# niqbal996/triton_client

Hardware: AMD Instinct MI355X
Metric: end-to-end FPS (sensor->detection) YOLOv5n-640 + PointPillars at 1/2/4/8 GPU (higher is better)
Workload: dtype fp32

## Files before the change

### csrc/kernels/conv_hx3.hip

```cpp
#include "tca_mfma.h"

#include <cstdlib>

using namespace tca;

namespace {

struct Hx3Args {
  const float* in_f;
  const float* res_f;
  float* out_f;
  const void* w;
  const float* bias;
  int B, H, W, Cin, ldi, ci_off, Ho, Wo;
  int N, ldo, co_off, ldr, r_off;
  int act;
  const unsigned char* occ;
  const unsigned char* uni;
  const float* uni_val;
  int uni_min;
};

template <int TH, int BN, int WM, int WN, bool CM>
__device__ __forceinline__ void hx3_epilogue(const Hx3Args& a, unsigned char* smem,
                                             const f32x4 (&acc)[TH / WM][BN / WN / 16], int b, int oy0, int ox0,
                                             int n0) {
  constexpr int BM = TH * 16, NT = WM * WN * 64, FM = TH / WM, FN = BN / WN / 16, LD = BN;
  static_assert(BN % 64 == 0, "the quad swizzle needs >= 16 quads per row");
  const int tid = threadIdx.x, lane = tid & 63, wid = tid >> 6;
  const int wm = wid / WN, wn = wid % WN, fr = lane & 15, fq = lane >> 4;
  float* st = reinterpret_cast<float*>(smem);
  auto quad = [](int ml, int q) { return ml * LD + ((q ^ (ml & 15)) << 2); };
  const int act = a.act & 15;
  const bool post_res = (a.act & 16) != 0 && a.res_f != nullptr;
  const int eact = post_res ? 0 : act;
#pragma unroll
  for (int j = 0; j < FN; ++j) {
    const int nl = (wn * FN + j) * 16 + fq * 4;
    const float4 bv = a.bias ? *reinterpret_cast<const float4*>(a.bias + n0 + nl) : make_float4(0.f, 0.f, 0.f, 0.f);
#pragma unroll
    for (int i = 0; i < FM; ++i) {
      const int ml = (wm * FM + i) * 16 + fr;
      float4 q = make_float4(acc[i][j][0] + bv.x, acc[i][j][1] + bv.y, acc[i][j][2] + bv.z, acc[i][j][3] + bv.w);
      if (eact == 1) {
        q.x = fmaxf(q.x, 0.f); q.y = fmaxf(q.y, 0.f); q.z = fmaxf(q.z, 0.f); q.w = fmaxf(q.w, 0.f);
      } else if (eact != 0) {
        q.x = act_fn(q.x, eact); q.y = act_fn(q.y, eact); q.z = act_fn(q.z, eact); q.w = act_fn(q.w, eact);
      }
      *reinterpret_cast<float4*>(st + quad(ml, nl >> 2)) = q;
    }
  }
  __syncthreads();
  constexpr int V8 = BN / 8;
  for (int id = tid; id < BM * V8; id += NT) {
    const int ml = id / V8, c8 = (id - (id / V8) * V8) * 8;
    const int oy = oy0 + (CM ? (ml & 15) : ml / 16), ox = ox0 + (CM ? ml / 16 : (ml & 15)), n = n0 + c8;
    if (oy >= a.Ho || ox >= a.Wo) continue;
    float v[8];
    const float4 v0 = *reinterpret_cast<const float4*>(st + quad(ml, c8 >> 2));
    const float4 v1 = *reinterpret_cast<const float4*>(st + quad(ml, (c8 >> 2) + 1));
    v[0] = v0.x; v[1] = v0.y; v[2] = v0.z; v[3] = v0.w; v[4] = v1.x; v[5] = v1.y; v[6] = v1.z; v[7] = v1.w;
    const long pix = ((long)b * a.Ho + oy) * a.Wo + ox;
    if (a.res_f) {
      float r[8];
      pair_join8(a.res_f + pix * a.ldr + a.r_off + n, r);
#pragma unroll
      for (int e = 0; e < 8; ++e) v[e] = post_res ? act_fn(v[e] + r[e], act) : v[e] + r[e];
    }
    const long o = pix * a.ldo + a.co_off + n;
    if (a.act & 32) {
      *reinterpret_cast<float4*>(a.out_f + o) = make_float4(v[0], v[1], v[2], v[3]);
      *reinterpret_cast<float4*>(a.out_f + o + 4) = make_float4(v[4], v[5], v[6], v[7]);
      continue;
    }
    uint4 hi, lo;
    pair_split8(v, hi, lo);
    *reinterpret_cast<uint4*>(a.out_f + o) = hi;
    *reinterpret_cast<uint4*>(a.out_f + o + 4) = lo;
  }
}

template <int BM, int BN, bool CM, int NT>
__device__ __forceinline__ bool uni_tile_store(const Hx3Args& a, int b, int oy0, int ox0, int n0) {
  const int tid = threadIdx.x;
  bool bad = false;
  for (int ml = tid; ml < BM; ml += NT) {
    const int oy = oy0 + (CM ? (ml & 15) : ml / 16), ox = ox0 + (CM ? ml / 16 : (ml & 15));
    if (oy < a.Ho && ox < a.Wo) bad |= a.uni[((long)b * a.Ho + oy) * a.Wo + ox] < a.uni_min;
  }
  if (__syncthreads_or(bad)) return false;
  constexpr int Q = BN / 4;
  for (int id = tid; id < BM * Q; id += NT) {
    const int ml = id / Q, q = id - (id / Q) * Q;
    const int oy = oy0 + (CM ? (ml & 15) : ml / 16), ox = ox0 + (CM ? ml / 16 : (ml & 15));
    if (oy >= a.Ho || ox >= a.Wo) continue;
    const long o = (((long)b * a.Ho + oy) * a.Wo + ox) * a.ldo + a.co_off + n0 + q * 4;
    *reinterpret_cast<uint4*>(a.out_f + o) = *reinterpret_cast<const uint4*>(a.uni_val + n0 + q * 4);
  }
  return true;
}

template <int V> struct IC { static constexpr int value = V; };

template <int TH, int BN, int WM, int WN, bool CM, int HB, int MINW = 2, bool PAIRS = false>
__global__ void __launch_bounds__(WM * WN * 64, MINW) conv_hx3_kernel(Hx3Args a) {
  constexpr int TW = 16, BM = TH * TW, NW = WM * WN, NT = NW * 64;
  constexpr int FM = TH / WM, FN = BN / WN / 16;
  static_assert(TH % WM == 0 && BN % (WN * 16) == 0 && FN >= 1, "tiles");
  static_assert(HB == 1 || HB == 2, "halo buffers");
  constexpr int HWD = TW + 2, HP = (TH + 2) * HWD;
  constexpr int HPIECES = HP * 8;
  constexpr int HPL = (HPIECES + NT - 1) / NT;
  constexpr int HBYTES = HP * 128;
  constexpr int EPI = BM * (BN + 4) * 4;
  constexpr int LDS = (HB * HBYTES > EPI) ? HB * HBYTES : EPI;
  __shared__ __attribute__((aligned(1024))) unsigned char smem[LDS];

  const int tid = threadIdx.x, lane = tid & 63, wid = tid >> 6;
  const int wm = wid / WN, wn = wid % WN;
  constexpr int EX = CM ? TH : TW, EY = CM ? TW : TH;
  const int tx_n = (a.Wo + EX - 1) / EX, ty_n = (a.Ho + EY - 1) / EY;
  const int nmt = a.B * ty_n * tx_n, nnt = a.N / BN, nwg = nmt * nnt;
  int bid = blockIdx.x;
  {
    const int xcd = bid & 7, q = nwg >> 3, r = nwg & 7;
    if (nwg >= 8) bid = (xcd < r ? xcd * (q + 1) : r * (q + 1) + (xcd - r) * q) + (bid >> 3);
  }
  const int mt = bid / nnt, nt = bid - mt * nnt;
  const int b = mt / (ty_n * tx_n), rem = mt - b * (ty_n * tx_n);
  const int oy0 = (rem / tx_n) * EY, ox0 = (rem - (rem / tx_n) * tx_n) * EX;
  const int n0 = nt * BN;

  if (a.uni && uni_tile_store<TH * TW, BN, CM, NT>(a, b, oy0, ox0, n0)) return;

  const __amdgpu_buffer_rsrc_t rin = __builtin_amdgcn_make_buffer_rsrc(
      (void*)a.in_f, (short)0, a.B * a.H * a.W * a.ldi * 4, 0x00020000);
  unsigned h_off[HPL];
  int h_lds[HPL];
#pragma unroll
  for (int k = 0; k < HPL; ++k) {
    const int q = tid + k * NT, p = q >> 3, piece = q & 7;
    h_off[k] = kOutOfRange;
    h_lds[k] = -1;
    if (q < HPIECES) {
      const int u = p / HWD, v = p - (p / HWD) * HWD;
      const int hy = CM ? v : u, hx = CM ? u : v;
      const int iy = oy0 - 1 + hy, ix = ox0 - 1 + hx;
      if ((unsigned)iy < (unsigned)a.H && (unsigned)ix < (unsigned)a.W)
        h_off[k] = (unsigned)((((b * a.H + iy) * a.W + ix) * a.ldi + a.ci_off) * 4 + piece * 16);
      h_lds[k] = p * 128 + ((piece ^ hswz(v)) << 4);
    }
  }
  typedef unsigned int u32x4 __attribute__((ext_vector_type(4)));
  u32x4 hreg[HPL];
  auto halo_load = [&](int c) {
#pragma unroll
    for (int k = 0; k < HPL; ++k) hreg[k] = __builtin_amdgcn_raw_buffer_load_b128(rin, h_off[k], c * 128, 0);
  };
  auto halo_write = [&](int buf) {
    unsigned char* dst = smem + buf * HBYTES;
#pragma unroll
    for (int k = 0; k < HPL; ++k)
      if (k + 1 < HPL || h_lds[k] >= 0) *reinterpret_cast<u32x4*>(dst + h_lds[k]) = hreg[k];
  };

  const int NG = a.N / 16, g0 = (n0 + wn * FN * 16) / 16;
  const __bf16* wf = reinterpret_cast<const __bf16*>(a.w) + (long)g0 * 1024 + lane * 8;
  const int nc = a.Cin / 32;
  auto wload = [&](int ks, bf16x8 (&dst)[FN][2]) {
    const __bf16* p = wf + (long)ks * NG * 1024;
#pragma unroll
    for (int j = 0; j < FN; ++j) {
      dst[j][0] = *reinterpret_cast<const bf16x8*>(p + j * 1024);
      dst[j][1] = *reinterpret_cast<const bf16x8*>(p + j * 1024 + 512);
    }
  };

  f32x4 acc[FM][FN];
#pragma unroll
  for (int i = 0; i < FM; ++i)
#pragma unroll
    for (int j = 0; j < FN; ++j) acc[i][j] = f32x4{0.f, 0.f, 0.f, 0.f};

  const int G = 3 * nc;
  auto gload = [&](int gs, bf16x8 (&dst)[3][FN][2]) {
    const int c = gs / 3, kf = gs - (gs / 3) * 3;
#pragma unroll
    for (int kl = 0; kl < 3; ++kl) {
      const int t = CM ? 3 * kf + kl : 3 * kl + kf;
      wload(t * nc + c, dst[kl]);
    }
  };
  bf16x8 wc[3][FN][2], wx[3][FN][2];
  halo_load(0);
  gload(0, wc);
  halo_write(0);
  halo_load(nc > 1 ? 1 : 0);
  asm volatile("s_waitcnt lgkmcnt(0)" ::: "memory");
  __builtin_amdgcn_s_barrier();
  asm volatile("" ::: "memory");

  const int fr = lane & 15, fq = lane >> 4;
  auto group = [&](auto KF, const unsigned char* hb, bf16x8 (&wu)[3][FN][2], bf16x8 (&wl)[3][FN][2], int gs_next) {
    constexpr int kf = decltype(KF)::value;
    gload(gs_next < G ? gs_next : G - 1, wl);
    __builtin_amdgcn_sched_barrier(0);
    const int sw = hswz(kf + fr);
    const unsigned char* colp = hb + (wm * FM) * HWD * 128 + (kf + fr) * 128;
    const int o_hi = ((2 * fq) ^ sw) << 4, o_lo = ((2 * fq + 1) ^ sw) << 4;
#pragma unroll
    for (int L = 0; L < FM + 2; ++L) {
      const bf16x8 ah = *reinterpret_cast<const bf16x8*>(colp + L * HWD * 128 + o_hi);
      const bf16x8 al = *reinterpret_cast<const bf16x8*>(colp + L * HWD * 128 + o_lo);
#pragma unroll
      for (int pr = 0; pr < 3; ++pr) {
#pragma unroll
        for (int kl = 0; kl < 3; ++kl) {
          const int i = L - kl;
          if (i < 0 || i >= FM) continue;
#pragma unroll
          for (int j = 0; j < FN; ++j) {
            const bf16x8& b = pr == 0 ? wu[kl][j][1] : wu[kl][j][0];
            const bf16x8& x = pr == 1 ? al : ah;
            acc[i][j] = __builtin_amdgcn_mfma_f32_16x16x32_bf16(b, x, acc[i][j], 0, 0, 0);
          }
        }
      }
    }
  };
  auto chunk_end = [&](int c) {
    if (c + 1 < nc) {
      if constexpr (HB == 1) {
        asm volatile("s_waitcnt lgkmcnt(0)" ::: "memory");
        __builtin_amdgcn_s_barrier();
        asm volatile("" ::: "memory");
      }
      halo_write(HB == 2 ? (c + 1) & 1 : 0);
      halo_load(c + 2 < nc ? c + 2 : nc - 1);
      asm volatile("s_waitcnt lgkmcnt(0)" ::: "memory");
      __builtin_amdgcn_s_barrier();
      asm volatile("" ::: "memory");
    }
  };
  if constexpr (PAIRS) {
    const unsigned char* hb1 = smem + (HB == 2 ? HBYTES : 0);
    for (int c = 0; c < nc; c += 2) {
      group(IC<0>{}, smem, wc, wx, 3 * c + 1);
      group(IC<1>{}, smem, wx, wc, 3 * c + 2);
      group(IC<2>{}, smem, wc, wx, 3 * c + 3);
      chunk_end(c);
      group(IC<0>{}, hb1, wx, wc, 3 * c + 4);
      group(IC<1>{}, hb1, wc, wx, 3 * c + 5);
      group(IC<2>{}, hb1, wx, wc, 3 * c + 6);
      chunk_end(c + 1);
    }
  } else {
    for (int c = 0; c < nc; ++c) {
      const unsigned char* hb = smem + (HB == 2 ? (c & 1) * HBYTES : 0);
      auto copyw = [&]() {
#pragma unroll
        for (int kl = 0; kl < 3; ++kl)
#pragma unroll
          for (int j = 0; j < FN; ++j) {
            wc[kl][j][0] = wx[kl][j][0];
            wc[kl][j][1] = wx[kl][j][1];
          }
      };
      group(IC<0>{}, hb, wc, wx, 3 * c + 1);
      copyw();
      group(IC<1>{}, hb, wc, wx, 3 * c + 2);
      copyw();
      group(IC<2>{}, hb, wc, wx, 3 * c + 3);
      copyw();
      chunk_end(c);
    }
  }
  asm volatile("s_waitcnt lgkmcnt(0)" ::: "memory");
  __builtin_amdgcn_s_barrier();
  asm volatile("" ::: "memory");

  hx3_epilogue<TH, BN, WM, WN, CM>(a, smem, acc, b, oy0, ox0, n0);
}

template <int G> struct S2Group {
  static constexpr int PL = G >= 3 ? 1 : 0;
  static constexpr int PF = (G == 0 || G == 3) ? 0 : 1;
  static constexpr int FI = (G == 2 || G == 5) ? 1 : 0;
  static constexpr int KF = PF == 0 ? 1 : 2 * FI;
  static constexpr int FOFF = PF == 0 ? 1 : FI;
  static constexpr int NL = PL == 0 ? 1 : 2;
  static constexpr int PH = PL * 2 + PF;
  static constexpr bool LAST_OF_PHASE = G == 0 || G == 2 || G == 3 || G == 5;
  __device__ static constexpr int kl(int li) { return PL == 0 ? 1 : 2 * li; }
  __device__ static constexpr int loff(int li) { return PL == 0 ? 1 : li; }
};

template <int TH, int BN, int WN, bool CM, int MINW, bool OCC>
__global__ void __launch_bounds__(WN * 64, MINW) conv_hx3s2_kernel(Hx3Args a) {
  constexpr int TW = 16, NT = WN * 64;
  constexpr int FM = TH, FN = BN / WN / 16;
  static_assert(BN % (WN * 16) == 0 && FN >= 1, "tiles");
  constexpr int HWD = TW + 1, HP = (TH + 1) * HWD;
  constexpr int HPIECES = HP * 8;
  constexpr int HPL = (HPIECES + NT - 1) / NT;
  constexpr int HBYTES = HP * 128;
  constexpr int EPI = TH * TW * (BN + 4) * 4;
  constexpr int LDS = (2 * HBYTES > EPI) ? 2 * HBYTES : EPI;
  __shared__ __attribute__((aligned(1024))) unsigned char smem[LDS];

  const int tid = threadIdx.x, lane = tid & 63, wn = tid >> 6;
  constexpr int EX = CM ? TH : TW, EY = CM ? TW : TH;
  const int tx_n = (a.Wo + EX - 1) / EX, ty_n = (a.Ho + EY - 1) / EY;
  const int nmt = a.B * ty_n * tx_n, nnt = a.N / BN, nwg = nmt * nnt;
  int bid = blockIdx.x;
  {
    const int xcd = bid & 7, q = nwg >> 3, r = nwg & 7;
    if (nwg >= 8) bid = (xcd < r ? xcd * (q + 1) : r * (q + 1) + (xcd - r) * q) + (bid >> 3);
  }
  const int mt = bid / nnt, nt = bid - mt * nnt;
  const int b = mt / (ty_n * tx_n), rem = mt - b * (ty_n * tx_n);
  const int oy0 = (rem / tx_n) * EY, ox0 = (rem - (rem / tx_n) * tx_n) * EX;
  const int n0 = nt * BN;
  if (a.uni && uni_tile_store<TH * TW, BN, CM, NT>(a, b, oy0, ox0, n0)) return;

  const __amdgpu_buffer_rsrc_t rin = __builtin_amdgcn_make_buffer_rsrc(
      (void*)a.in_f, (short)0, a.B * a.H * a.W * a.ldi * 4, 0x00020000);
  const int pix_b = a.ldi * 4, row_b = a.W * a.ldi * 4;
  const int dl = CM ? pix_b : row_b, df = CM ? row_b : pix_b;
  unsigned h_off[HPL];
  int h_lds[HPL];
  unsigned h_ph[HPL];
#pragma unroll
  for (int k = 0; k < HPL; ++k) {
    const int q = tid + k * NT, p = q >> 3, piece = q & 7;
    h_off[k] = kOutOfRange;
    h_lds[k] = -1;
    h_ph[k] = 0;
    if (q < HPIECES) {
      const int u = p / HWD, v = p - (p / HWD) * HWD;
      const int hy = CM ? v : u, hx = CM ? u : v;
      const int Y = oy0 - 1 + hy, X = ox0 - 1 + hx;
      if (Y >= 0 && X >= 0 && 2 * Y < a.H && 2 * X < a.W) {
        h_off[k] = (unsigned)((((b * a.H + 2 * Y) * a.W + 2 * X) * a.ldi + a.ci_off) * 4 + piece * 16);
#pragma unroll
        for (int ph = 0; ph < 4; ++ph) {
          const int pl = ph >> 1, pf = ph & 1;
          const int iy = 2 * Y + (CM ? pf : pl), ix = 2 * X + (CM ? pl : pf);
          bool ok = iy < a.H && ix < a.W;
          if constexpr (OCC) ok = ok && a.occ[((long)b * a.H + iy) * a.W + ix] != 0;
          h_ph[k] |= ok ? (1u << ph) : 0u;
        }
      }
      h_lds[k] = p * 128 + ((piece ^ hswz(v)) << 4);
    }
  }
  typedef unsigned int u32x4 __attribute__((ext_vector_type(4)));
  u32x4 hreg[2][HPL];
  auto halo_load = [&](int ph, int c, auto SL) {
    constexpr int sl = decltype(SL)::value;
    const int so = c * 128 + (ph >> 1) * dl + (ph & 1) * df;
#pragma unroll
    for (int k = 0; k < HPL; ++k)
      hreg[sl][k] = __builtin_amdgcn_raw_buffer_load_b128(rin, ((h_ph[k] >> ph) & 1u) ? h_off[k] : kOutOfRange, so, 0);
  };
  auto halo_write = [&](int buf, auto SL) {
    constexpr int sl = decltype(SL)::value;
    unsigned char* dst = smem + buf * HBYTES;
#pragma unroll
    for (int k = 0; k < HPL; ++k)
      if (k + 1 < HPL || h_lds[k] >= 0) *reinterpret_cast<u32x4*>(dst + h_lds[k]) = hreg[sl][k];
  };

  const int NG = a.N / 16, g0 = (n0 + wn * FN * 16) / 16;
  const __bf16* wf = reinterpret_cast<const __bf16*>(a.w) + (long)g0 * 1024 + lane * 8;
  const int nc = a.Cin / 32;
  auto wload = [&](int ks, bf16x8 (&dst)[FN][2]) {
    const __bf16* p = wf + (long)ks * NG * 1024;
#pragma unroll
    for (int j = 0; j < FN; ++j) {
      dst[j][0] = *reinterpret_cast<const bf16x8*>(p + j * 1024);
      dst[j][1] = *reinterpret_cast<const bf16x8*>(p + j * 1024 + 512);
    }
  };
  auto gload = [&](auto GC, int c, bf16x8 (&dst)[2][FN][2]) {
    using S = S2Group<decltype(GC)::value>;
#pragma unroll
    for (int li = 0; li < S::NL; ++li) {
      const int t = CM ? 3 * S::KF + S::kl(li) : 3 * S::kl(li) + S::KF;
      wload(t * nc + c, dst[li]);
    }
  };

  f32x4 acc[FM][FN];
#pragma unroll
  for (int i = 0; i < FM; ++i)
#pragma unroll
    for (int j = 0; j < FN; ++j) acc[i][j] = f32x4{0.f, 0.f, 0.f, 0.f};

  if constexpr (OCC) {
    unsigned mine = 0;
#pragma unroll
    for (int k = 0; k < HPL; ++k) mine |= h_ph[k];
    if (!__syncthreads_or(mine != 0u)) {
      hx3_epilogue<TH, BN, 1, WN, CM>(a, smem, acc, b, oy0, ox0, n0);
      return;
    }
  }
  bf16x8 w0[2][FN][2], w1[2][FN][2];
  halo_load(0, 0, IC<0>{});
  gload(IC<0>{}, 0, w0);
  halo_write(0, IC<0>{});
  halo_load(1, 0, IC<1>{});
  halo_load(4 * nc > 2 ? 2 : 4 * nc - 1, 0, IC<0>{});
  asm volatile("s_waitcnt lgkmcnt(0)" ::: "memory");
  __builtin_amdgcn_s_barrier();
  asm volatile("" ::: "memory");

  const int fr = lane & 15, fq = lane >> 4;
  auto phase_end = [&](auto PH, int c) {
    constexpr int ph = decltype(PH)::value;
    const int q = 4 * c + ph;
    if (q + 1 < 4 * nc) {
      halo_write((ph + 1) & 1, IC<(ph + 1) & 1>{});
      const int q3 = q + 3 < 4 * nc ? q + 3 : 4 * nc - 1;
      halo_load(q3 & 3, q3 >> 2, IC<(ph + 1) & 1>{});
      asm volatile("s_waitcnt lgkmcnt(0)" ::: "memory");
      __builtin_amdgcn_s_barrier();
      asm volatile("" ::: "memory");
    }
  };
  auto group = [&](auto GC, int c, bf16x8 (&wu)[2][FN][2], bf16x8 (&wl)[2][FN][2]) {
    constexpr int G = decltype(GC)::value;
    using S = S2Group<G>;
    if constexpr (G < 5) gload(IC<G + 1>{}, c, wl);
    else gload(IC<0>{}, c + 1 < nc ? c + 1 : nc - 1, wl);
    __builtin_amdgcn_sched_barrier(0);
    const unsigned char* hb = smem + (S::PH & 1) * HBYTES;
    const int sw = hswz(S::FOFF + fr);
    const unsigned char* colp = hb + (S::FOFF + fr) * 128;
    const int o_hi = ((2 * fq) ^ sw) << 4, o_lo = ((2 * fq + 1) ^ sw) << 4;
#pragma unroll
    for (int L = (S::NL == 1 ? 1 : 0); L < FM + 1; ++L) {
      const bf16x8 ah = *reinterpret_cast<const bf16x8*>(colp + L * HWD * 128 + o_hi);
      const bf16x8 al = *reinterpret_cast<const bf16x8*>(colp + L * HWD * 128 + o_lo);
#pragma unroll
      for (int pr = 0; pr < 3; ++pr) {
#pragma unroll
        for (int li = 0; li < S::NL; ++li) {
          const int i = L - S::loff(li);
          if (i < 0 || i >= FM) continue;
#pragma unroll
          for (int j = 0; j < FN; ++j) {
            const bf16x8& b = pr == 0 ? wu[li][j][1] : wu[li][j][0];
            const bf16x8& x = pr == 1 ? al : ah;
            acc[i][j] = __builtin_amdgcn_mfma_f32_16x16x32_bf16(b, x, acc[i][j], 0, 0, 0);
          }
        }
      }
    }
    if constexpr (S::LAST_OF_PHASE) phase_end(IC<S::PH>{}, c);
  };
  for (int c = 0; c < nc; ++c) {
    group(IC<0>{}, c, w0, w1);
    group(IC<1>{}, c, w1, w0);
    group(IC<2>{}, c, w0, w1);
    group(IC<3>{}, c, w1, w0);
    group(IC<4>{}, c, w0, w1);
    group(IC<5>{}, c, w1, w0);
  }
  asm volatile("s_waitcnt lgkmcnt(0)" ::: "memory");
  __builtin_amdgcn_s_barrier();
  asm volatile("" ::: "memory");
  hx3_epilogue<TH, BN, 1, WN, CM>(a, smem, acc, b, oy0, ox0, n0);
}


template <int TH, int BN, int WM, int WN, bool CM, int HB, int MINW = 2>
int launch_hx3(const Hx3Args& a, hipStream_t stream) {
  if (a.N % BN) return (int)hipErrorInvalidValue;
  const int ex = CM ? TH : 16, ey = CM ? 16 : TH;
  const int nwg = a.B * ((a.Ho + ey - 1) / ey) * ((a.Wo + ex - 1) / ex) * (a.N / BN);
  if ((a.Cin / 32) % 2 == 0)
    conv_hx3_kernel<TH, BN, WM, WN, CM, HB, MINW, true><<<nwg, WM * WN * 64, 0, stream>>>(a);
  else
    conv_hx3_kernel<TH, BN, WM, WN, CM, HB, MINW, false><<<nwg, WM * WN * 64, 0, stream>>>(a);
  return (int)hipGetLastError();
}

int hx3_launch(const Hx3Args& a, int tile, hipStream_t stream) {
  if (tile == 0) {
    const long rm8 = (long)((a.Wo + 15) / 16 * 16) * ((a.Ho + 7) / 8 * 8);
    const long cm8 = (long)((a.Ho + 15) / 16 * 16) * ((a.Wo + 7) / 8 * 8);
    if (a.N % 128 == 0) tile = cm8 < rm8 ? 2 : 1;
    else if (a.N % 64 == 0) tile = cm8 < rm8 ? 6 : 5;
    else return (int)hipErrorInvalidValue;
  }
  switch (tile) {
    case 1: return launch_hx3<8, 128, 1, 4, false, 2>(a, stream);
    case 2: return launch_hx3<8, 128, 1, 4, true, 2>(a, stream);
    case 3: return launch_hx3<8, 64, 2, 2, false, 2>(a, stream);
    case 4: return launch_hx3<8, 64, 2, 2, true, 2>(a, stream);
    case 5: return launch_hx3<8, 64, 1, 4, false, 2, 3>(a, stream);
    case 6: return launch_hx3<8, 64, 1, 4, true, 2, 3>(a, stream);
    default: return (int)hipErrorInvalidValue;
  }
}


template <int TH, int BN, int WN, bool CM, int MINW>
int launch_hx3s2(const Hx3Args& a, hipStream_t stream) {
  if (a.N % BN) return (int)hipErrorInvalidValue;
  const int ex = CM ? TH : 16, ey = CM ? 16 : TH;
  const int nwg = a.B * ((a.Ho + ey - 1) / ey) * ((a.Wo + ex - 1) / ex) * (a.N / BN);
  if (a.occ) conv_hx3s2_kernel<TH, BN, WN, CM, MINW, true><<<nwg, WN * 64, 0, stream>>>(a);
  else conv_hx3s2_kernel<TH, BN, WN, CM, MINW, false><<<nwg, WN * 64, 0, stream>>>(a);
  return (int)hipGetLastError();
}

int hx3s2_launch(const Hx3Args& a, int tile, hipStream_t stream) {
  if (tile == 0) {
    const long rm8 = (long)((a.Wo + 15) / 16 * 16) * ((a.Ho + 7) / 8 * 8);
    const long cm8 = (long)((a.Ho + 15) / 16 * 16) * ((a.Wo + 7) / 8 * 8);
    if (a.N % 128 == 0) tile = cm8 < rm8 ? 2 : 1;
    else if (a.N % 64 == 0) tile = cm8 < rm8 ? 4 : 3;
    else return (int)hipErrorInvalidValue;
  }
  switch (tile) {
    case 1: return launch_hx3s2<8, 128, 4, false, 2>(a, stream);
    case 2: return launch_hx3s2<8, 128, 4, true, 2>(a, stream);
    case 3: return launch_hx3s2<8, 64, 4, false, 3>(a, stream);
    case 4: return launch_hx3s2<8, 64, 4, true, 3>(a, stream);
    default: return (int)hipErrorInvalidValue;
  }
}

}

TCA_API int tca_conv_hx3p(const float* in, int B, int H, int W, int Cin, int ldi, int ci_off, const void* wfrag,
                          const float* bias, int N, float* out, int ldo, int co_off, int act, const float* res,
                          int ldr, int r_off, int tile, hipStream_t stream) {
  if (B <= 0) return 0;
  if ((Cin & 31) || (ldi & 7) || (ci_off & 7) || (N & 63) || (ldo & 7) || (co_off & 7)) return (int)hipErrorInvalidValue;
  if (res && ((ldr & 7) || (r_off & 7))) return (int)hipErrorInvalidValue;
  Hx3Args a;
  a.in_f = in; a.res_f = res; a.out_f = out; a.w = wfrag; a.bias = bias; a.occ = nullptr;
  a.uni = nullptr; a.uni_val = nullptr; a.uni_min = 0;
  a.B = B; a.H = H; a.W = W; a.Cin = Cin; a.ldi = ldi; a.ci_off = ci_off; a.Ho = H; a.Wo = W;
  a.N = N; a.ldo = ldo; a.co_off = co_off; a.ldr = ldr; a.r_off = r_off; a.act = act;
  if ((long)B * H * W * ldi * 4 >= (1L << 31)) return (int)hipErrorInvalidValue;
  return hx3_launch(a, tile, stream);
}

TCA_API int tca_conv_hx3s2p(const float* in, int B, int H, int W, int Cin, int ldi, int ci_off, const void* wfrag,
                            const float* bias, int N, float* out, int ldo, int co_off, int act, const float* res,
                            int ldr, int r_off, const unsigned char* occ, const unsigned char* uni, int uni_min,
                            const float* uni_val, int tile, hipStream_t stream) {
  if (B <= 0) return 0;
  if ((act & 32) && res) return (int)hipErrorInvalidValue;
  if ((Cin & 31) || (ldi & 7) || (ci_off & 7) || (N & 63) || (ldo & 7) || (co_off & 7)) return (int)hipErrorInvalidValue;
  if (res && ((ldr & 7) || (r_off & 7))) return (int)hipErrorInvalidValue;
  Hx3Args a;
  if (uni && (!uni_val || uni_min < 1 || res)) return (int)hipErrorInvalidValue;
  a.in_f = in; a.res_f = res; a.out_f = out; a.w = wfrag; a.bias = bias; a.occ = occ;
  a.uni = uni; a.uni_val = uni_val; a.uni_min = uni ? uni_min : 0;
  a.B = B; a.H = H; a.W = W; a.Cin = Cin; a.ldi = ldi; a.ci_off = ci_off; a.Ho = (H + 1) / 2; a.Wo = (W + 1) / 2;
  a.N = N; a.ldo = ldo; a.co_off = co_off; a.ldr = ldr; a.r_off = r_off; a.act = act;
  if ((long)B * H * W * ldi * 4 >= (1L << 31)) return (int)hipErrorInvalidValue;
  return hx3s2_launch(a, tile, stream);
}

TCA_API int tca_conv_hx3p_uni(const float* in, int B, int H, int W, int Cin, int ldi, int ci_off, const void* wfrag,
                              const float* bias, int N, float* out, int ldo, int co_off, int act,
                              const unsigned char* uni, int uni_min, const float* uni_val, int tile,
                              hipStream_t stream) {
  if (B <= 0) return 0;
  if ((Cin & 31) || (ldi & 7) || (ci_off & 7) || (N & 63) || (ldo & 7) || (co_off & 7)) return (int)hipErrorInvalidValue;
  if (!uni || !uni_val || uni_min < 1) return (int)hipErrorInvalidValue;
  Hx3Args a;
  a.in_f = in; a.res_f = nullptr; a.out_f = out; a.w = wfrag; a.bias = bias; a.occ = nullptr;
  a.uni = uni; a.uni_val = uni_val; a.uni_min = uni_min;
  a.B = B; a.H = H; a.W = W; a.Cin = Cin; a.ldi = ldi; a.ci_off = ci_off; a.Ho = H; a.Wo = W;
  a.N = N; a.ldo = ldo; a.co_off = co_off; a.ldr = 0; a.r_off = 0; a.act = act;
  if ((long)B * H * W * ldi * 4 >= (1L << 31)) return (int)hipErrorInvalidValue;
  return hx3_launch(a, tile, stream);
}

namespace {

constexpr int UD_TY = 16, UD_TX = 64, UD_MAXR = 7;
static_assert(UD_TX + 2 * UD_MAXR < 128, "u rows are walked 128 columns at a time");

__global__ void __launch_bounds__(256) bev_uniform_depth_kernel(const unsigned char* __restrict__ occ, int H, int W,
                                                                 int Ho, int Wo, int maxd,
                                                                 unsigned char* __restrict__ depth) {
  constexpr int LY = UD_TY + 2 * UD_MAXR, LX = UD_TX + 2 * UD_MAXR;
  constexpr int OY = 2 * LY + 1, OX = 2 * LX + 1;
  __shared__ unsigned char u[LY * LX];
  __shared__ unsigned char os[OY * OX];
  const int b = blockIdx.z, ty0 = blockIdx.y * UD_TY, tx0 = blockIdx.x * UD_TX;
  const int R = maxd - 1;
  const int ry = UD_TY + 2 * R, rx = UD_TX + 2 * R;
  const unsigned char* oc = occ + (long)b * H * W;
  const int iy0 = 2 * (ty0 - R) - 1, ix0 = 2 * (tx0 - R) - 1, oy = 2 * ry + 1, ox = 2 * rx + 1;
  const int lane = threadIdx.x & 63, wv = threadIdx.x >> 6, nw = blockDim.x >> 6;
  for (int r = wv; r < oy; r += nw) {
    const int iy = iy0 + r;
    const bool row_in = (unsigned)iy < (unsigned)H;
    for (int c = lane; c < ox; c += 64) {
      const int ix = ix0 + c;
      os[r * OX + c] = (row_in && (unsigned)ix < (unsigned)W) ? oc[(long)iy * W + ix] : 0;
    }
  }
  __syncthreads();
  for (int id = threadIdx.x; id < ry * 128; id += blockDim.x) {
    const int ly = id >> 7, lx = id & 127;
    if (lx >= rx) continue;
    const int Y = ty0 - R + ly, X = tx0 - R + lx;
    unsigned char good = 0;
    if (Y >= 0 && X >= 0 && Y < Ho && X < Wo) {
      const unsigned char* w = os + (2 * ly) * OX + 2 * lx;
      const unsigned any = w[0] | w[1] | w[2] | w[OX] | w[OX + 1] | w[OX + 2] | w[2 * OX] | w[2 * OX + 1] |
                           w[2 * OX + 2];
      good = any ? 0 : 1;
    }
    u[ly * LX + lx] = good;
  }
  __syncthreads();
  for (int id = threadIdx.x; id < UD_TY * UD_TX; id += blockDim.x) {
    const int py = id / UD_TX, px = id - (id / UD_TX) * UD_TX;
    const int Y = ty0 + py, X = tx0 + px;
    if (Y >= Ho || X >= Wo) continue;
    const int cy = py + R, cx = px + R;
    int d = 0;
    if (u[cy * LX + cx]) {
      d = 1;
      for (int k = 1; k <= R; ++k) {
        bool ok = true;
        for (int t = -k; t <= k && ok; ++t)
          ok = u[(cy - k) * LX + cx + t] && u[(cy + k) * LX + cx + t] && u[(cy + t) * LX + cx - k] &&
               u[(cy + t) * LX + cx + k];
        if (!ok) break;
        d = k + 1;
      }
    }
    depth[((long)b * Ho + Y) * Wo + X] = (unsigned char)d;
  }
}

}

TCA_API int tca_bev_uniform_depth(const unsigned char* occ, int B, int H, int W, int maxd, unsigned char* depth,
                                  hipStream_t stream) {
  if (B <= 0) return 0;
  if (maxd < 1 || maxd > UD_MAXR + 1) return (int)hipErrorInvalidValue;
  const int Ho = (H + 1) / 2, Wo = (W + 1) / 2;
  dim3 grid((unsigned)((Wo + UD_TX - 1) / UD_TX), (unsigned)((Ho + UD_TY - 1) / UD_TY), (unsigned)B);
  bev_uniform_depth_kernel<<<grid, 256, 0, stream>>>(occ, H, W, Ho, Wo, maxd, depth);
  TCA_LAUNCH_CHECK();
}
```

### triton_client_amd/ops/conv.py

```python
from __future__ import annotations

import os

from dataclasses import dataclass
from typing import Optional

import torch
import torch.nn as nn
import torch.nn.functional as F

from .. import _native
from ..models.common import ACT_LEAKY, ACT_NONE, ACT_RELU, ACT_SILU, apply_act


@dataclass
class NHWC:
    t: torch.Tensor
    off: int = 0
    c: Optional[int] = None
    pair: bool = False
    occ: Optional[torch.Tensor] = None

    def __post_init__(self):
        if self.c is None:
            self.c = self.t.shape[-1] - self.off
        if self.pair:
            assert self.t.dtype == torch.float32 and self.off % 8 == 0 and self.c % 8 == 0, (self.off, self.c)

    @property
    def shape(self):
        return (*self.t.shape[:3], self.c)

    def tensor(self) -> torch.Tensor:
        return self.t[..., self.off:self.off + self.c]

    def slice(self, off: int, c: int) -> "NHWC":
        return NHWC(self.t, self.off + off, c, self.pair)

    def values(self) -> torch.Tensor:
        return from_pairs(self.tensor()) if self.pair else self.tensor()

    def nchw(self) -> torch.Tensor:
        return self.values().permute(0, 3, 1, 2)


def to_pairs(x: torch.Tensor) -> torch.Tensor:
    *lead, C = x.shape
    assert C % 8 == 0, C
    v = x.float().reshape(*lead, C // 8, 1, 8)
    hi = v.to(torch.bfloat16)
    lo = (v - hi.float()).to(torch.bfloat16)
    return torch.cat([hi, lo], -2).reshape(*lead, 2 * C).view(torch.float32)


def from_pairs(p: torch.Tensor) -> torch.Tensor:
    *lead, C = p.shape
    assert C % 8 == 0, C
    h = p.contiguous().view(torch.bfloat16).reshape(*lead, C // 8, 2, 8).float()
    return (h[..., 0, :] + h[..., 1, :]).reshape(*lead, C)


def _ceil(x, m):
    return (x + m - 1) // m * m


PRECISIONS = ("fp32", "bf16")
PAIR_TILES = (20, 22, 24, 25, 26, 32, 37, 41, 42, 68, 69, 70, 71, 72, 73, 74, 75, 76, 77, 78, 79, 90, 91, 92, 93, 94, 95, 96, 97, 102)


HX3 = True
HX3S2 = True
WINO = os.environ.get("TCA_WINO", "1") != "0"
WINO_MIN_N = int(os.environ.get("TCA_WINO_MIN_N", "128"))
S2SP = os.environ.get("TCA_S2SP", "0") == "1"
S2SP_TILE = int(os.environ.get("TCA_S2SP_TILE", "0"))
HX3_TILE_AUTO = int(os.environ.get("TCA_HX3_TILE", "0"))
HX3S2_TILE_AUTO = int(os.environ.get("TCA_HX3S2_TILE", "0"))
WINO_TILE_AUTO = int(os.environ.get("TCA_WINO_TILE", "0"))
TILES = {**{110 + t: ("hx3", t) for t in range(7)}, **{120 + t: ("hx3s2", t) for t in range(5)},
         **{130 + t: ("wino", t) for t in range(5)}, **{140 + t: ("s2sp", t) for t in range(3)},
         **{t: ("x3p", t) for t in PAIR_TILES}}
ENTRIES = {"bf16": "tca_conv_nhwc", "x3": "tca_conv_nhwc_x3", "x3p": "tca_conv_nhwc_x3p",
           "x3p_occ": "tca_conv_nhwc_x3p_occ", "hx3": "tca_conv_hx3p", "hx3_uni": "tca_conv_hx3p_uni",
           "hx3s2": "tca_conv_hx3s2p", "wino": "tca_conv_wino", "s2sp": "tca_conv_s2sp"}


@dataclass(frozen=True)
class Route:
    family: str
    tile: int
    out_fp32: bool = False
    gated: bool = False


def wino_tile(H: int, W: int, N: int) -> int:
    cm = (H + 31) // 32 * 32 * W <= (W + 31) // 32 * 32 * H
    return (2 if cm else 1) if N % 128 == 0 else (4 if cm else 3)


def wino_taps(W: torch.Tensor, cin: int, cm: bool) -> torch.Tensor:
    N = W.shape[0]
    g = W[:, :9 * cin].double().reshape(N, 3, 3, cin)
    if cm:
        g = g.permute(0, 2, 1, 3)
    g0, g1, g2 = g[:, :, 0], g[:, :, 1], g[:, :, 2]
    return torch.stack([g0, (g0 + g1 + g2) / 2, (g0 - g1 + g2) / 2, g2], 2)


def wino_weights(W: torch.Tensor, cin: int, cm: bool) -> torch.Tensor:
    N = W.shape[0]
    return frag_weights(wino_taps(W, cin, cm).reshape(N, 12 * cin).float())


def frag_weights(W: torch.Tensor) -> torch.Tensor:
    N, Kp = W.shape
    assert N % 16 == 0 and Kp % 32 == 0, (N, Kp)
    hi, lo = split_bf16(W)
    t = torch.stack([hi, lo], 0).reshape(2, N // 16, 16, Kp // 32, 4, 8)
    return t.permute(3, 1, 0, 4, 2, 5).contiguous()


def act_dtype(precision: str) -> torch.dtype:
    if precision not in PRECISIONS:
        raise ValueError(f"precision must be one of {PRECISIONS}, got {precision!r}")
    return torch.float32 if precision == "fp32" else torch.bfloat16


def split_bf16(w: torch.Tensor):
    w = w.float()
    hi = w.to(torch.bfloat16)
    lo = (w - hi.float()).to(torch.bfloat16)
    return hi, lo


def split_pairs(w: torch.Tensor) -> torch.Tensor:
    N, K = w.shape
    assert K % 8 == 0, K
    hi, lo = split_bf16(w)
    return torch.stack([hi.reshape(N, K // 8, 8), lo.reshape(N, K // 8, 8)], 2).reshape(N, 2 * K).contiguous()


def nhwc_dtype_code(t: torch.Tensor) -> int:
    if t.dtype == torch.float32:
        return 0
    if t.dtype == torch.bfloat16:
        return 2
    raise TypeError(f"NHWC activations must be fp32 or bf16, got {t.dtype}")


class FusedConv:
    def __init__(self, conv: nn.Module, act: int = ACT_NONE, device="cuda", cin_pad: Optional[int] = None,
                 cout_pad: Optional[int] = None, post_res: bool = False, precision: str = "bf16"):
        w = conv.weight.detach().float()
        b = conv.bias.detach().float() if conv.bias is not None else None
        self.transpose = isinstance(conv, nn.ConvTranspose2d)
        self.device = torch.device(device)
        self.act = act
        self.post_res = post_res
        self.precision = precision
        self.dtype = act_dtype(precision)
        if self.transpose:
            cin, cout, kh, kw = w.shape
            s = conv.stride[0]
            assert kh == kw == s and conv.padding[0] == 0, "only k == stride transpose convs"
            self.shuffle, self.k, self.s, self.p = s, 1, 1, 0
            self.cout_real = cout
            wg = w.permute(2, 3, 1, 0).reshape(s * s * cout, cin)
            bias = b.repeat(s * s) if b is not None else None
            self.ref = conv
        else:
            cout, cin, kh, kw = w.shape
            assert kh == kw
            self.shuffle, self.k, self.s, self.p = 0, kh, conv.stride[0], conv.padding[0]
            self.cout_real = cout
            wg = w
            bias = b
            self.ref = conv
        self.cin = cin
        self.cin_p = cin_pad or _ceil(cin, 8)
        if self.transpose:
            wk = torch.zeros(wg.shape[0], self.cin_p)
            wk[:, :cin] = wg
            K = self.cin_p
        else:
            wk = torch.zeros(cout, kh, kw, self.cin_p)
            wk[..., :cin] = wg.permute(0, 2, 3, 1)
            wk = wk.reshape(cout, -1)
            K = kh * kw * self.cin_p
        N = wk.shape[0]
        self.N = cout_pad or _ceil(N, 8)
        self.K, self.Kp = K, _ceil(K, 32)
        W = torch.zeros(self.N, self.Kp)
        W[:N, :K] = wk
        self.bias = torch.zeros(self.N)
        if bias is not None:
            self.bias[:N] = bias
        self.w_f32_gemm = W
        if precision == "fp32":
            self.w_gemm = split_pairs(W).to(self.device)
        else:
            self.w_gemm = W.to(self.device, torch.bfloat16).contiguous()
        self.b_gemm = self.bias.to(self.device).contiguous()
        self._w_frag = frag_weights(W).to(self.device) if self.hx3_ok() and self.device.type == "cuda" else None
        self._w_wino = {}
        self.w_f32, self.b_f32 = w, b

    def out_hw(self, H, W):
        if self.transpose:
            return H * self.shuffle, W * self.shuffle
        return (H + 2 * self.p - self.k) // self.s + 1, (W + 2 * self.p - self.k) // self.s + 1

    def out_channels(self) -> int:
        return self.cout_real if self.transpose else self.N

    def __call__(self, x: NHWC, out: Optional[NHWC] = None, res: Optional[NHWC] = None, tile: int = 0,
                 stream=None, uni=None) -> NHWC:
        B, H, W, C = x.shape
        Ho, Wo = self.out_hw(H, W)
        if out is None:
            out = NHWC(torch.empty((B, Ho, Wo, self.out_channels()), dtype=self.dtype, device=x.t.device))
        if x.t.device.type != "cuda":
            return self._cpu(x, out, res)
        assert C == self.cin_p, (C, self.cin_p)
        for t in (x.t, out.t) + ((res.t,) if res is not None else ()):
            if t.dtype != self.dtype:
                raise TypeError(f"{self.precision} conv needs {self.dtype} activations, got {t.dtype}")
        r = self.route(x.pair, out.pair, None if res is None else "pair" if res.pair else "fp32",
                       x.occ is not None, uni is not None, tile, H, W)
        act = self.act | (16 if (self.post_res and res is not None) else 0)
        getattr(self, "_" + r.family)(r, x, out, res, act, uni, _native.stream_ptr(stream))
        return out

    def route(self, x_pair: bool, out_pair: bool, res: Optional[str] = None, occ: bool = False, uni: bool = False,
              tile: int = 0, H: int = 0, W: int = 0) -> Route:
        assert res in (None, "pair", "fp32"), res
        fam, t = TILES.get(tile, (None, 0))
        if (not occ and res is None and self.wino_ok()) and (fam == "wino" or (tile == 0 and WINO)):
            return Route("wino", (t if fam == "wino" else 0) or WINO_TILE_AUTO or wino_tile(H, W, self.N),
                         out_fp32=not out_pair)
        if not (x_pair or out_pair):
            return Route("x3" if self.precision == "fp32" else "bf16", tile)
        if self.precision != "fp32" or not x_pair or (res is not None and (res == "pair") != out_pair):
            raise TypeError("pair activations: fp32 convs reading pairs (output pairs or fp32)")
        if (res is None and occ and self.s2sp_ok()) and (fam == "s2sp" or (tile == 0 and S2SP)):
            return Route("s2sp", t if fam == "s2sp" else S2SP_TILE, out_fp32=not out_pair, gated=True)
        if ((out_pair or res is None) and self.hx3_ok() and self.s == 2) and (fam == "hx3s2" or (tile == 0 and HX3S2)):
            return Route("hx3s2", t if fam == "hx3s2" else HX3S2_TILE_AUTO, out_fp32=not out_pair, gated=occ)
        if (out_pair and not occ and self.hx3_ok() and self.s == 1) and (fam == "hx3" or (tile == 0 and HX3)):
            return Route("hx3_uni" if uni and res is None else "hx3", t if fam == "hx3" else HX3_TILE_AUTO)
        gate = occ and not self.transpose
        return Route("x3p_occ" if gate else "x3p", t if fam == "x3p" else 0, gated=gate and self.k * self.k <= 32)

    def hx3_ok(self) -> bool:
        return (self.precision == "fp32" and not self.transpose and self.k == 3 and self.s in (1, 2) and self.p == 1
                and self.cin_p % 32 == 0 and self.K == self.Kp and self.N % 64 == 0)

    def wino_ok(self) -> bool:
        return self.hx3_ok() and self.s == 1 and self.act in (ACT_NONE, ACT_RELU) and self.N >= WINO_MIN_N

    @staticmethod
    def _in_args(x: NHWC):
        B, H, W, C = x.shape
        return _native.ptr(x.t), B, H, W, C, x.t.shape[-1], x.off

    @staticmethod
    def _res_args(res: Optional[NHWC]):
        return (_native.ptr(res.t), res.t.shape[-1], res.off) if res is not None else (_native.ptr(None), 0, 0)

    @staticmethod
    def _occ_ptr(x: NHWC) -> int:
        if x.occ is not None:
            assert x.occ.dtype == torch.uint8 and tuple(x.occ.shape) == tuple(x.shape[:3]), (x.occ.shape, x.shape)
        return _native.ptr(x.occ)

    def _uni_args(self, uni, x: NHWC):
        if uni is None:
            return _native.ptr(None), 0, _native.ptr(None)
        depth, dmin, val = uni
        assert depth.dtype == torch.uint8 and tuple(depth.shape) == (x.shape[0], *self.out_hw(*x.shape[1:3])), depth.shape
        assert val.dtype == torch.float32 and val.numel() == self.N, (val.dtype, val.shape)
        return _native.ptr(depth), dmin, _native.ptr(val)

    def _x3(self, r, x, out, res, act, uni, stream):
        H, W = x.shape[1:3]
        gh, gw = (H, W) if self.transpose else self.out_hw(H, W)
        tail = {"x3p": (int(out.pair),), "x3p_occ": (int(out.pair), self._occ_ptr(x))}.get(r.family, ())
        _native.call(ENTRIES[r.family], *self._in_args(x), _native.ptr(self.w_gemm), _native.ptr(self.b_gemm), self.N,
                     self.k, self.k, self.s, self.p, self.Kp, _native.ptr(out.t), gh, gw, out.t.shape[-1], out.off, act,
                     *self._res_args(res), self.shuffle, r.tile, *tail, stream)

    _bf16 = _x3p = _x3p_occ = _x3

    def _hx_args(self, x, out, act):
        return (*self._in_args(x), _native.ptr(self.hx3_weights()), _native.ptr(self.b_gemm), self.N,
                _native.ptr(out.t), out.t.shape[-1], out.off, act | (0 if out.pair else 32))

    def _s2sp(self, r, x, out, res, act, uni, stream):
        _native.call(ENTRIES[r.family], *self._hx_args(x, out, act), self._occ_ptr(x), r.tile, stream)

    def _hx3s2(self, r, x, out, res, act, uni, stream):
        _native.call(ENTRIES[r.family], *self._hx_args(x, out, act), *self._res_args(res), self._occ_ptr(x),
                     *self._uni_args(uni if res is None else None, x), r.tile, stream)

    def _hx3(self, r, x, out, res, act, uni, stream):
        mid = self._uni_args(uni, x) if r.family == "hx3_uni" else self._res_args(res)
        _native.call(ENTRIES[r.family], *self._hx_args(x, out, act), *mid, r.tile, stream)

    _hx3_uni = _hx3

    def _wino(self, r, x, out, res, act, uni, stream):
        cm = r.tile in (2, 4)
        wf = self._w_wino.get(cm)
        if wf is None:
            wf = self._w_wino[cm] = wino_weights(self.w_f32_gemm, self.cin_p, cm).to(self.device)
        _native.call(ENTRIES[r.family], *self._in_args(x), int(x.pair), _native.ptr(wf), _native.ptr(self.b_gemm),
                     self.N, _native.ptr(out.t), out.t.shape[-1], out.off, int(out.pair), act,
                     *self._uni_args(uni, x), r.tile, stream)

    def hx3_weights(self) -> torch.Tensor:
        if self._w_frag is None:
            self._w_frag = frag_weights(self.w_f32_gemm).to(self.device)
        return self._w_frag

    def s2sp_ok(self) -> bool:
        return (self.precision == "fp32" and not self.transpose and self.k == 3 and self.s == 2 and self.p == 1
                and self.N == 64 and self.cin_p in (32, 64) and self.K == self.Kp
                and self.act in (ACT_NONE, ACT_RELU, ACT_SILU, ACT_LEAKY))

    def pair_ok(self) -> bool:
        return self.precision == "fp32" and self.cin_p % 32 == 0 and self.K == self.Kp

    def _cpu(self, x: NHWC, out: NHWC, res: Optional[NHWC]) -> NHWC:
        xi = x.nchw().float()[:, : self.cin]
        if self.transpose:
            y = F.conv_transpose2d(xi, self.w_f32, self.b_f32, stride=self.shuffle)
        else:
            y = F.conv2d(xi, self.w_f32, self.b_f32, stride=self.s, padding=self.p)
        if res is not None and self.post_res:
            y = apply_act(y + res.nchw().float()[:, : y.shape[1]], self.act)
        else:
            y = apply_act(y, self.act)
            if res is not None:
                y = y + res.nchw().float()[:, : y.shape[1]]
        out.tensor()[..., : y.shape[1]].copy_(y.permute(0, 2, 3, 1).to(out.t.dtype))
        return out


def sppf_pools(y0: NHWC, dst: torch.Tensor, cs: int, k: int = 5, stream=None) -> None:
    B, H, W, C = y0.shape
    e = 4 if y0.t.dtype == torch.float32 else 8
    if (y0.t.is_cuda and C % (4 * e) == 0 and 2 * H * W * 64 <= 64 * 1024 and y0.off % e == 0
            and y0.t.shape[-1] % e == 0 and dst.shape[-1] % e == 0 and cs % e == 0):
        _native.call("tca_sppf_pool3", _native.ptr(y0.t), B, H, W, C, y0.t.shape[-1], y0.off, k, _native.ptr(dst),
                     dst.shape[-1], cs, 2 * cs, 3 * cs, nhwc_dtype_code(y0.t), _native.stream_ptr(stream))
        return
    y1 = maxpool_nhwc(y0, NHWC(dst, cs, cs), k, stream)
    y2 = maxpool_nhwc(y1, NHWC(dst, 2 * cs, cs), k, stream)
    maxpool_nhwc(y2, NHWC(dst, 3 * cs, cs), k, stream)


def maxpool_nhwc(x: NHWC, out: NHWC, k: int = 5, stream=None) -> NHWC:
    B, H, W, C = x.shape
    if x.t.device.type != "cuda":
        y = F.max_pool2d(x.nchw().float(), k, 1, k // 2)
        out.tensor().copy_(y.permute(0, 2, 3, 1).to(out.t.dtype))
        return out
    _native.call("tca_maxpool_nhwc", _native.ptr(x.t), B, H, W, C, x.t.shape[-1], x.off, k, _native.ptr(out.t),
                 out.t.shape[-1], out.off, nhwc_dtype_code(x.t), _native.stream_ptr(stream))
    return out


def maxpool2d_nhwc(x: NHWC, out: NHWC, k: int = 3, s: int = 2, p: int = 1, stream=None) -> NHWC:
    B, H, W, C = x.shape
    Ho, Wo = out.shape[1], out.shape[2]
    if x.t.device.type != "cuda":
        y = F.max_pool2d(x.nchw().float(), k, s, p)
        out.tensor().copy_(y.permute(0, 2, 3, 1).to(out.t.dtype))
        return out
    _native.call("tca_maxpool2d_nhwc", _native.ptr(x.t), B, H, W, C, x.t.shape[-1], x.off, k, s, p,
                 _native.ptr(out.t), Ho, Wo, out.t.shape[-1], out.off, nhwc_dtype_code(x.t), _native.stream_ptr(stream))
    return out


def upsample2x_nhwc(x: NHWC, out: NHWC, stream=None) -> NHWC:
    B, H, W, C = x.shape
    if x.t.device.type != "cuda":
        y = F.interpolate(x.nchw().float(), scale_factor=2.0, mode="nearest")
        out.tensor().copy_(y.permute(0, 2, 3, 1).to(out.t.dtype))
        return out
    _native.call("tca_upsample2x_nhwc", _native.ptr(x.t), B, H, W, C, x.t.shape[-1], x.off, _native.ptr(out.t),
                 out.t.shape[-1], out.off, nhwc_dtype_code(x.t), _native.stream_ptr(stream))
    return out
```

Before: 5081.

## Stage all four stride-2 phases per channel chunk in LDS for hx3s2 conv

Adds a window-staging variant of the stride-2 3x3 conv kernel that holds all four input phases of a 32-channel chunk in LDS at once. The next chunk's halo loads are spread across groups 2-5, and there is one swap per chunk instead of a barrier at the end of each phase. This aims to cut per-phase barrier and LDS write stalls. In exchange it doubles LDS use for halo buffers and adds registers for four halo slots, which may lower occupancy. The auto tile selection picks it for dense inputs with N divisible by 128 and Cin >= 128.

```diff
diff --git a/csrc/kernels/conv_hx3.hip b/csrc/kernels/conv_hx3.hip
--- a/csrc/kernels/conv_hx3.hip
+++ b/csrc/kernels/conv_hx3.hip
@@ -295,17 +295,19 @@
   __device__ static constexpr int loff(int li) { return PL == 0 ? 1 : li; }
 };
 
-template <int TH, int BN, int WN, bool CM, int MINW, bool OCC>
+template <int TH, int BN, int WN, bool CM, int MINW, bool OCC, bool WIN = false>
 __global__ void __launch_bounds__(WN * 64, MINW) conv_hx3s2_kernel(Hx3Args a) {
   constexpr int TW = 16, NT = WN * 64;
   constexpr int FM = TH, FN = BN / WN / 16;
   static_assert(BN % (WN * 16) == 0 && FN >= 1, "tiles");
+  static_assert(!(WIN && OCC), "window staging: dense input only");
+  constexpr int NB = WIN ? 4 : 2;
   constexpr int HWD = TW + 1, HP = (TH + 1) * HWD;
   constexpr int HPIECES = HP * 8;
   constexpr int HPL = (HPIECES + NT - 1) / NT;
   constexpr int HBYTES = HP * 128;
   constexpr int EPI = TH * TW * (BN + 4) * 4;
-  constexpr int LDS = (2 * HBYTES > EPI) ? 2 * HBYTES : EPI;
+  constexpr int LDS = (NB * HBYTES > EPI) ? NB * HBYTES : EPI;
   __shared__ __attribute__((aligned(1024))) unsigned char smem[LDS];
 
   const int tid = threadIdx.x, lane = tid & 63, wn = tid >> 6;
@@ -354,14 +356,26 @@
       h_lds[k] = p * 128 + ((piece ^ hswz(v)) << 4);
     }
   }
+  static_assert(!WIN || (HPL <= 8 && NT % 8 == 0), "packed piece bits");
+  unsigned h_phs = 0, h_sws = 0;
+  if constexpr (WIN) {
+#pragma unroll
+    for (int k = 0; k < HPL; ++k) {
+      h_phs |= h_ph[k] << (4 * k);
+      h_sws |= (unsigned)((h_lds[k] >> 4) & 7) << (3 * k);
+    }
+  }
   typedef unsigned int u32x4 __attribute__((ext_vector_type(4)));
-  u32x4 hreg[2][HPL];
-  auto halo_load = [&](int ph, int c, auto SL) {
+  u32x4 hreg[NB][HPL];
+  auto halo_load = [&](int ph, int c, auto SL, bool live = true) {
     constexpr int sl = decltype(SL)::value;
     const int so = c * 128 + (ph >> 1) * dl + (ph & 1) * df;
-#pragma unroll
-    for (int k = 0; k < HPL; ++k)
-      hreg[sl][k] = __builtin_amdgcn_raw_buffer_load_b128(rin, ((h_ph[k] >> ph) & 1u) ? h_off[k] : kOutOfRange, so, 0);
+    const unsigned m = live ? 1u << ph : 0u;
+#pragma unroll
+    for (int k = 0; k < HPL; ++k) {
+      const bool in = WIN ? (h_phs & (m << (4 * k))) != 0u : ((h_ph[k] >> ph) & 1u) != 0u;
+      hreg[sl][k] = __builtin_amdgcn_raw_buffer_load_b128(rin, in ? h_off[k] : kOutOfRange, so, 0);
+    }
   };
   auto halo_write = [&](int buf, auto SL) {
     constexpr int sl = decltype(SL)::value;
@@ -369,6 +383,17 @@
 #pragma unroll
     for (int k = 0; k < HPL; ++k)
       if (k + 1 < HPL || h_lds[k] >= 0) *reinterpret_cast<u32x4*>(dst + h_lds[k]) = hreg[sl][k];
+  };
+  auto window_write = [&]() {
+    unsigned sws = h_sws;
+    asm volatile("" : "+v"(sws));
+#pragma unroll
+    for (int k = 0; k < HPL; ++k) {
+      if (k + 1 == HPL && tid + k * NT >= HPIECES) continue;
+      unsigned char* dst = smem + ((tid + k * NT) >> 3) * 128 + (((sws >> (3 * k)) & 7u) << 4);
+#pragma unroll
+      for (int ph = 0; ph < NB; ++ph) *reinterpret_cast<u32x4*>(dst + ph * HBYTES) = hreg[ph][k];
+    }
   };
 
   const int NG = a.N / 16, g0 = (n0 + wn * FN * 16) / 16;
@@ -407,11 +432,20 @@
     }
   }
   bf16x8 w0[2][FN][2], w1[2][FN][2];
-  halo_load(0, 0, IC<0>{});
-  gload(IC<0>{}, 0, w0);
-  halo_write(0, IC<0>{});
-  halo_load(1, 0, IC<1>{});
-  halo_load(4 * nc > 2 ? 2 : 4 * nc - 1, 0, IC<0>{});
+  if constexpr (WIN) {
+    halo_load(0, 0, IC<0>{});
+    halo_load(1, 0, IC<1>{});
+    halo_load(2, 0, IC<2>{});
+    halo_load(3, 0, IC<3>{});
+    gload(IC<0>{}, 0, w0);
+    window_write();
+  } else {
+    halo_load(0, 0, IC<0>{});
+    gload(IC<0>{}, 0, w0);
+    halo_write(0, IC<0>{});
+    halo_load(1, 0, IC<1>{});
+    halo_load(4 * nc > 2 ? 2 : 4 * nc - 1, 0, IC<0>{});
+  }
   asm volatile("s_waitcnt lgkmcnt(0)" ::: "memory");
   __builtin_amdgcn_s_barrier();
   asm volatile("" ::: "memory");
@@ -429,13 +463,27 @@
       asm volatile("" ::: "memory");
     }
   };
+  auto window_swap = [&](int c) {
+    if constexpr (WIN) {
+      if (c + 1 < nc) {
+        asm volatile("s_waitcnt lgkmcnt(0)" ::: "memory");
+        __builtin_amdgcn_s_barrier();
+        asm volatile("" ::: "memory");
+        window_write();
+        asm volatile("s_waitcnt lgkmcnt(0)" ::: "memory");
+        __builtin_amdgcn_s_barrier();
+        asm volatile("" ::: "memory");
+      }
+    }
+  };
   auto group = [&](auto GC, int c, bf16x8 (&wu)[2][FN][2], bf16x8 (&wl)[2][FN][2]) {
     constexpr int G = decltype(GC)::value;
     using S = S2Group<G>;
     if constexpr (G < 5) gload(IC<G + 1>{}, c, wl);
     else gload(IC<0>{}, c + 1 < nc ? c + 1 : nc - 1, wl);
+    if constexpr (WIN && G >= 2) halo_load(G - 2, c + 1, IC<G - 2>{}, c + 1 < nc);
     __builtin_amdgcn_sched_barrier(0);
-    const unsigned char* hb = smem + (S::PH & 1) * HBYTES;
+    const unsigned char* hb = smem + (WIN ? S::PH : S::PH & 1) * HBYTES;
     const int sw = hswz(S::FOFF + fr);
     const unsigned char* colp = hb + (S::FOFF + fr) * 128;
     const int o_hi = ((2 * fq) ^ sw) << 4, o_lo = ((2 * fq + 1) ^ sw) << 4;
@@ -458,7 +506,11 @@
         }
       }
     }
-    if constexpr (S::LAST_OF_PHASE) phase_end(IC<S::PH>{}, c);
+    if constexpr (WIN) {
+      if constexpr (G == 5) window_swap(c);
+    } else if constexpr (S::LAST_OF_PHASE) {
+      phase_end(IC<S::PH>{}, c);
+    }
   };
   for (int c = 0; c < nc; ++c) {
     group(IC<0>{}, c, w0, w1);
@@ -507,13 +559,18 @@
 }
 
 
-template <int TH, int BN, int WN, bool CM, int MINW>
+template <int TH, int BN, int WN, bool CM, int MINW, bool WIN = false>
 int launch_hx3s2(const Hx3Args& a, hipStream_t stream) {
   if (a.N % BN) return (int)hipErrorInvalidValue;
   const int ex = CM ? TH : 16, ey = CM ? 16 : TH;
   const int nwg = a.B * ((a.Ho + ey - 1) / ey) * ((a.Wo + ex - 1) / ex) * (a.N / BN);
-  if (a.occ) conv_hx3s2_kernel<TH, BN, WN, CM, MINW, true><<<nwg, WN * 64, 0, stream>>>(a);
-  else conv_hx3s2_kernel<TH, BN, WN, CM, MINW, false><<<nwg, WN * 64, 0, stream>>>(a);
+  if constexpr (WIN) {
+    if (a.occ) return (int)hipErrorInvalidValue;
+    conv_hx3s2_kernel<TH, BN, WN, CM, MINW, false, true><<<nwg, WN * 64, 0, stream>>>(a);
+  } else {
+    if (a.occ) conv_hx3s2_kernel<TH, BN, WN, CM, MINW, true><<<nwg, WN * 64, 0, stream>>>(a);
+    else conv_hx3s2_kernel<TH, BN, WN, CM, MINW, false><<<nwg, WN * 64, 0, stream>>>(a);
+  }
   return (int)hipGetLastError();
 }
 
@@ -521,7 +578,7 @@
   if (tile == 0) {
     const long rm8 = (long)((a.Wo + 15) / 16 * 16) * ((a.Ho + 7) / 8 * 8);
     const long cm8 = (long)((a.Ho + 15) / 16 * 16) * ((a.Wo + 7) / 8 * 8);
-    if (a.N % 128 == 0) tile = cm8 < rm8 ? 2 : 1;
+    if (a.N % 128 == 0) tile = (cm8 < rm8 ? 2 : 1) + ((!a.occ && !a.uni && a.Cin >= 128) ? 4 : 0);
     else if (a.N % 64 == 0) tile = cm8 < rm8 ? 4 : 3;
     else return (int)hipErrorInvalidValue;
   }
@@ -530,6 +587,8 @@
     case 2: return launch_hx3s2<8, 128, 4, true, 2>(a, stream);
     case 3: return launch_hx3s2<8, 64, 4, false, 3>(a, stream);
     case 4: return launch_hx3s2<8, 64, 4, true, 3>(a, stream);
+    case 5: return launch_hx3s2<8, 128, 4, false, 2, true>(a, stream);
+    case 6: return launch_hx3s2<8, 128, 4, true, 2, true>(a, stream);
     default: return (int)hipErrorInvalidValue;
   }
 }
diff --git a/triton_client_amd/ops/conv.py b/triton_client_amd/ops/conv.py
--- a/triton_client_amd/ops/conv.py
+++ b/triton_client_amd/ops/conv.py
@@ -77,7 +77,7 @@
 HX3_TILE_AUTO = int(os.environ.get("TCA_HX3_TILE", "0"))
 HX3S2_TILE_AUTO = int(os.environ.get("TCA_HX3S2_TILE", "0"))
 WINO_TILE_AUTO = int(os.environ.get("TCA_WINO_TILE", "0"))
-TILES = {**{110 + t: ("hx3", t) for t in range(7)}, **{120 + t: ("hx3s2", t) for t in range(5)},
+TILES = {**{110 + t: ("hx3", t) for t in range(7)}, **{120 + t: ("hx3s2", t) for t in range(7)},
          **{130 + t: ("wino", t) for t in range(5)}, **{140 + t: ("s2sp", t) for t in range(3)},
          **{t: ("x3p", t) for t in PAIR_TILES}}
 ENTRIES = {"bf16": "tca_conv_nhwc", "x3": "tca_conv_nhwc_x3", "x3p": "tca_conv_nhwc_x3p",
```

Result: no change. 5053 (-0.5%).
